# Advanced-Vision-and-Learning-Lab/sparse-view-3dgs-pack

Hardware: AMD Instinct MI355X
Metric: train-step views/s (fwd+bwd) @1M Gaussians 1080p (higher is better)
Workload: dtype f32

## Files before the change

profiles/summarize.py:

```python
#!/usr/bin/env python3
import collections
import csv
import glob
import json
import os
import sys

src, tag = sys.argv[1], sys.argv[2]
script_dir = os.path.dirname(os.path.abspath(__file__))
here = sys.argv[3] if len(sys.argv) > 3 else script_dir
sys.path.insert(0, script_dir)
from source_id import source_id


def run_identity():
    ident = {"tag": tag, "source_id": source_id(os.path.dirname(script_dir))}
    try:
        line = [x for x in open(os.path.join(src, "bench_trace.json")).read().splitlines() if x.startswith("{")][-1]
        j = json.loads(line)
        ident["P"] = j["config"]["gaussians"]
        ident["R"] = j["config"]["num_rendered_last_view"]
        ident["workload"] = j["config"]["workload"]
    except Exception as e:
        ident["identity_error"] = repr(e)
    return ident
OURS = ("preprocess_fwd_kernel", "scan_block_sums_kernel", "rs_hist_kernel", "rs_scatter_kernel", "scan_reduce_kernel",
        "scan_sums_kernel", "scan_down_kernel", "rs_rowscan_kernel", "sorted_block_sums_kernel", "duplicate_kernel", "tile_ranges_kernel",
        "bin_prepare_kernel", "render_fwd_wave_kernel", "render_bwd_wave_kernel", "render_fwd_kernel", "render_bwd_kernel", "adam_kernel", "scan_small_kernel", "preprocess_bwd_kernel", "l1_fwd_kernel",
        "l1_bwd_kernel", "dwt2_l1_fwd_kernel", "dwt2_l1_bwd_kernel", "ssim_fwd_kernel", "ssim_bwd_kernel",
        "patch_dwt_kernel", "lgdwt_combine_kernel", "act_fwd_kernel", "act_bwd_kernel", "densify_stats_kernel", "patch_means_kernel", "elf_low_kernel", "bilinear_up_kernel", "knn_search_kernel", "preprocess_bwd_step_kernel",
        "tile_order_kernel", "zero_rows_kernel", "stop_depth_bounds_kernel", "region_bin_kernel", "region_prepare_kernel",
        "status_tag_kernel", "rs_small_sort_kernel", "step_uninstanced_kernel", "chain_kernel",
        "tb_entries_kernel", "tb_emit_kernel", "tb_regions_from_counts_kernel", "tb_regions_kernel", "tb_tile_count_kernel",
        "tb_region_scan_kernel", "tb_tile_scan_kernel", "tb_write_kernel", "depth_l1_kernel", "rows_pack_kernel", "row_mask_kernel",
        "ssim_fwd_clamp_kernel", "lgdwt_bwd_kernel")


def short(name):
    for o in sorted(OURS, key=len, reverse=True):
        if o in name:
            return o
    return name.split("(")[0][-60:]


stats = glob.glob(os.path.join(src, "trace", "*", "*_kernel_stats.csv"))[0]
rows = list(csv.DictReader(open(stats)))
import shutil
shutil.copyfile(stats, os.path.join(here, "%s_rocprofv3_kernel_stats_full.csv" % tag))
with open(os.path.join(here, "%s_kernel_stats.csv" % tag), "w") as f:
    w = csv.writer(f)
    w.writerow(["Name", "Calls", "TotalDurationNs", "AverageNs", "Percentage", "MinNs", "MaxNs"])
    for r in rows[:40]:
        w.writerow([short(r["Name"]), r["Calls"], r["TotalDurationNs"], r["AverageNs"], r["Percentage"], r["MinNs"], r["MaxNs"]])

trace = glob.glob(os.path.join(src, "trace", "*", "*_kernel_trace.csv"))[0]
tr = sorted(csv.DictReader(open(trace)), key=lambda r: int(r["Start_Timestamp"]))
idx = [i for i, r in enumerate(tr) if "render_bwd_wave_kernel" in r["Kernel_Name"] or "render_bwd_kernel" in r["Kernel_Name"]]
a, b = idx[-3], idx[-2]
for j in range(len(idx) - 2, 0, -1):
    if any("step_uninstanced_kernel" in r["Kernel_Name"] for r in tr[idx[j - 1]:idx[j]]):
        a, b = idx[j - 1], idx[j]
        break
seg = tr[a:b]
wall = (int(tr[b]["Start_Timestamp"]) - int(seg[0]["Start_Timestamp"])) / 1e6
t_end = int(tr[b]["Start_Timestamp"])
iv = sorted((int(r["Start_Timestamp"]), min(int(r["End_Timestamp"]), t_end)) for r in seg)
busy, cur_s, cur_e = 0.0, None, None
for s0, e0 in iv:
    if cur_e is None or s0 > cur_e:
        if cur_e is not None:
            busy += cur_e - cur_s
        cur_s, cur_e = s0, e0
    else:
        cur_e = max(cur_e, e0)
busy = (busy + (cur_e - cur_s if cur_e is not None else 0)) / 1e6
agg = collections.OrderedDict()
for r in seg:
    n = short(r["Kernel_Name"])
    agg.setdefault(n, [0.0, 0])
    agg[n][0] += (int(r["End_Timestamp"]) - int(r["Start_Timestamp"])) / 1e3
    agg[n][1] += 1
with open(os.path.join(here, "%s_step_timeline.txt" % tag), "w") as f:
    f.write("one steady-state train step (render_bwd to render_bwd), rocprofv3 --kernel-trace\n")
    f.write("wall %.3f ms, GPU busy %.3f ms, %d kernel launches\n" % (wall, busy, len(seg)))
    for n, (d, c) in sorted(agg.items(), key=lambda x: -x[1][0]):
        f.write("%10.1f us %4d  %s\n" % (d, c, n))

traffic = {}
table = collections.defaultdict(lambda: {"FETCH_SIZE": [], "WRITE_SIZE": []})
for kind in ("fetch", "write"):
    files = glob.glob(os.path.join(src, kind, "*", "*_counter_collection.csv"))
    if not files:
        continue
    for r in csv.DictReader(open(files[0])):
        table[short(r["Kernel_Name"])][r["Counter_Name"]].append(float(r["Counter_Value"]))
with open(os.path.join(here, "%s_pmc_traffic.csv" % tag), "w") as f:
    w = csv.writer(f)
    w.writerow(["kernel", "launches", "FETCH_SIZE_KiB_mean", "WRITE_SIZE_KiB_mean", "hbm_read_bytes_corrected(x2)",
                "hbm_write_bytes", "hbm_total_bytes_per_launch"])
    for k, v in sorted(table.items()):
        if k not in OURS or not v["FETCH_SIZE"]:
            continue
        fs = v["FETCH_SIZE"][-max(1, len(v["FETCH_SIZE"]) // 3):]
        ws = v["WRITE_SIZE"][-max(1, len(v["WRITE_SIZE"]) // 3):] if v["WRITE_SIZE"] else [0.0]
        fm, wm = sum(fs) / len(fs), sum(ws) / len(ws)
        rd, wr = 2.0 * fm * 1024.0, wm * 1024.0
        w.writerow([k, len(v["FETCH_SIZE"]), "%.1f" % fm, "%.1f" % wm, "%.0f" % rd, "%.0f" % wr, "%.0f" % (rd + wr)])
        traffic[k] = rd + wr
stage_of = {"render_bwd": "render_bwd_wave_kernel", "render_fwd": "render_fwd_wave_kernel", "preprocess_fwd": "preprocess_fwd_kernel",
            "preprocess_bwd": "preprocess_bwd_kernel", "preprocess_bwd_step": "preprocess_bwd_step_kernel",
            "duplicate": "duplicate_kernel", "tile_ranges": "tile_ranges_kernel", "region_bin": "region_bin_kernel",
            "ssim_fwd": "ssim_fwd_kernel", "ssim_bwd": "ssim_bwd_kernel",
            "step_uninstanced": "step_uninstanced_kernel", "chain": "chain_kernel"}
for st, kn in (("ssim_fwd", "ssim_fwd_clamp_kernel"), ("ssim_bwd", "lgdwt_bwd_kernel")):
    if kn in traffic:
        stage_of[st] = kn
out = {st: traffic[k] for st, k in stage_of.items() if k in traffic}
out.update(run_identity())
out["launches_counted"] = {st: len(table[k]["FETCH_SIZE"]) for st, k in stage_of.items() if k in traffic}
if "region_bin_kernel" in traffic:
    out["sort"] = traffic["region_bin_kernel"]
elif "rs_scatter_kernel" in traffic:
    out["sort"] = 6 * (traffic.get("rs_scatter_kernel", 0) + traffic.get("rs_hist_kernel", 0))
json.dump(out, open(os.path.join(here, "pmc_traffic.json"), "w"), indent=1)
print(open(os.path.join(here, "%s_step_timeline.txt" % tag)).read())
print(open(os.path.join(here, "%s_pmc_traffic.csv" % tag)).read())

sq = collections.defaultdict(lambda: collections.defaultdict(list))
for f in glob.glob(os.path.join(src, "sq[0-9]*", "*", "*_counter_collection.csv")):
    for r in csv.DictReader(open(f)):
        sq[short(r["Kernel_Name"])][r["Counter_Name"]].append(float(r["Counter_Value"]))
if sq:
    with open(os.path.join(here, "%s_sq_counters.csv" % tag), "w") as f:
        w = csv.writer(f)
        w.writerow(["kernel", "waves", "VALU_insts_per_wave", "LDS_insts_per_wave", "SALU_insts_per_wave", "VMEM_rd_per_wave",
                    "VMEM_wr_per_wave", "VALU_issue_pct_of_peak", "VALU_active_x4_pct_of_SIMD_cycles", "wait_any_pct_of_wave_cycles",
                    "wait_inst_pct_of_wave_cycles", "waves_per_SIMD", "LDS_bank_conflict_pct_of_LDS_cycles"])
        sq_insts = run_identity()
        sq_insts["launches_counted"] = {}
        for k, v in sorted(sq.items()):
            m = {c: sum(x) / len(x) for c, x in v.items()}
            if k not in OURS or "GRBM_GUI_ACTIVE" not in m or m.get("SQ_WAVES", 0) == 0:
                continue
            simd_cycles = m["GRBM_GUI_ACTIVE"] / 8 * 1024
            wc = max(1.0, m.get("SQ_WAVE_CYCLES", 0))
            w.writerow([k, int(m["SQ_WAVES"]), round(m.get("SQ_INSTS_VALU", 0) / m["SQ_WAVES"], 1),
                        round(m.get("SQ_INSTS_LDS", 0) / m["SQ_WAVES"], 1), round(m.get("SQ_INSTS_SALU", 0) / m["SQ_WAVES"], 1),
                        round(m.get("SQ_INSTS_VMEM_RD", 0) / m["SQ_WAVES"], 1), round(m.get("SQ_INSTS_VMEM_WR", 0) / m["SQ_WAVES"], 1),
                        round(100 * m.get("SQ_INSTS_VALU", 0) * 2 / simd_cycles, 1),
                        round(100 * m.get("SQ_ACTIVE_INST_VALU", 0) * 4 / simd_cycles, 1),
                        round(100 * m.get("SQ_WAIT_ANY", 0) / wc, 1), round(100 * m.get("SQ_WAIT_INST_ANY", 0) / wc, 1),
                        round(wc * 4 / simd_cycles, 2),
                        round(100 * m.get("SQ_LDS_BANK_CONFLICT", 0) / max(1.0, m.get("SQ_LDS_IDX_ACTIVE", 0)), 1)])
            for st, kn in (("render_bwd", "render_bwd_wave_kernel"), ("render_fwd", "render_fwd_wave_kernel")):
                if k == kn:
                    sq_insts[st] = m.get("SQ_INSTS_VALU", 0)
                    sq_insts["launches_counted"][st] = len(v.get("SQ_INSTS_VALU", []))
                    sq_insts[st + "_valu_active_cycles_per_simd"] = m.get("SQ_ACTIVE_INST_VALU", 0) * 4 / 1024
                    sq_insts[st + "_valu_active_share_under_profiler"] = m.get("SQ_ACTIVE_INST_VALU", 0) * 4 / simd_cycles
    json.dump(sq_insts, open(os.path.join(here, "sq_insts.json"), "w"), indent=1)
    print(open(os.path.join(here, "%s_sq_counters.csv" % tag)).read())


for kind in ("init_like",):
    st_files = glob.glob(os.path.join(src, "trace_" + kind, "*", "*_kernel_stats.csv"))
    if not st_files:
        continue
# ... 66 lines not shown
```

sparse-view-3dgs-pack_amd/csrc/gs_loss.hip:

```cpp
#include "gs_common.h"
#include "gs_prof.h"

#define HC 0.7071067811865476f

struct Bands {
  float ll, lh, hl, hh;
};
__device__ __forceinline__ Bands haar_block(float a, float b, float c, float d) {
  const float lo_t = HC * a + HC * b, hi_t = HC * a - HC * b;
  const float lo_b = HC * c + HC * d, hi_b = HC * c - HC * d;
  Bands r;
  r.ll = HC * lo_t + HC * lo_b;
  r.lh = HC * lo_t - HC * lo_b;
  r.hl = HC * hi_t + HC * hi_b;
  r.hh = HC * hi_t - HC * hi_b;
  return r;
}
__device__ __forceinline__ void haar_block_adj(float gll, float glh, float ghl, float ghh, float& da, float& db,
                                               float& dc, float& dd) {
  const float dlo_t = HC * gll + HC * glh, dlo_b = HC * gll - HC * glh;
  const float dhi_t = HC * ghl + HC * ghh, dhi_b = HC * ghl - HC * ghh;
  da = HC * dlo_t + HC * dhi_t;
  db = HC * dlo_t - HC * dhi_t;
  dc = HC * dlo_b + HC * dhi_b;
  dd = HC * dlo_b - HC * dhi_b;
}
__device__ __forceinline__ float sgnf(float x) { return (float)((x > 0.f) - (x < 0.f)); }
__device__ __forceinline__ int cdiv2(int n) { return (n + 1) >> 1; }

template <int N>
__device__ __forceinline__ void block_sum_atomic(float (&v)[N], float* out) {
  __shared__ float red[GS_BLOCK / 64][N];
#pragma unroll
  for (int k = 0; k < N; k++) {
    float x = v[k];
#pragma unroll
    for (int off = 32; off >= 1; off >>= 1) x += __shfl_down(x, off, 64);
    if ((threadIdx.x & 63) == 0) red[threadIdx.x >> 6][k] = x;
  }
  __syncthreads();
  if (threadIdx.x < N) {
    float s = 0.f;
    for (int w = 0; w < GS_BLOCK / 64; w++) s += red[w][threadIdx.x];
    if (s != 0.f) atomicAdd(&out[threadIdx.x], s);
  }
}

__global__ void __launch_bounds__(GS_BLOCK) l1_fwd_kernel(const float* __restrict__ a, const float* __restrict__ b,
                                                          int64_t n, float* sum, float* __restrict__ partials) {
  float acc[1] = {0.f};
  const int64_t n4 = n >> 2;
  const float4* a4 = reinterpret_cast<const float4*>(a);
// ... 92 lines not shown
    } else if (!py && pxp) {
      p[(size_t)y0 * W + x0] = da + db;
      p[(size_t)(y0 + 1) * W + x0] = dc + dd;
    } else {
      p[(size_t)y0 * W + x0] = ((da + db) + dc) + dd;
    }
  }
}

struct Px44 {
  float v[4][4];
};
struct Blk44 {
  float l1[2][2][4];
  float l2[4];
};
template <bool FAST>
__device__ __forceinline__ void load_px44(const float* __restrict__ p, int H, int W, int i2, int j2, int h1, int w1,
                                          Px44& o) {
  if (FAST) {
#pragma unroll
    for (int y = 0; y < 4; y++) {
      const float4 q = reinterpret_cast<const float4*>(p + (size_t)(4 * i2 + y) * W)[j2];
      o.v[y][0] = q.x; o.v[y][1] = q.y; o.v[y][2] = q.z; o.v[y][3] = q.w;
    }
  } else {
#pragma unroll
    for (int r = 0; r < 2; r++)
#pragma unroll
      for (int c = 0; c < 2; c++) {
        const int r1 = min(2 * i2 + r, h1 - 1), c1 = min(2 * j2 + c, w1 - 1);
        const int y0 = 2 * r1, y1 = min(2 * r1 + 1, H - 1), x0 = 2 * c1, x1 = min(2 * c1 + 1, W - 1);
        o.v[2 * r][2 * c] = p[(size_t)y0 * W + x0];
        o.v[2 * r][2 * c + 1] = p[(size_t)y0 * W + x1];
        o.v[2 * r + 1][2 * c] = p[(size_t)y1 * W + x0];
        o.v[2 * r + 1][2 * c + 1] = p[(size_t)y1 * W + x1];
      }
  }
}
__device__ __forceinline__ void bands_of(const Px44& x, Blk44& o) {
  float ll[2][2];
#pragma unroll
  for (int r = 0; r < 2; r++)
#pragma unroll
    for (int c = 0; c < 2; c++) {
      const Bands b = haar_block(x.v[2 * r][2 * c], x.v[2 * r][2 * c + 1], x.v[2 * r + 1][2 * c], x.v[2 * r + 1][2 * c + 1]);
      o.l1[r][c][0] = b.ll; o.l1[r][c][1] = b.lh; o.l1[r][c][2] = b.hl; o.l1[r][c][3] = b.hh;
      ll[r][c] = b.ll;
    }
  const Bands b2 = haar_block(ll[0][0], ll[0][1], ll[1][0], ll[1][1]);
  o.l2[0] = b2.ll; o.l2[1] = b2.lh; o.l2[2] = b2.hl; o.l2[3] = b2.hh;
}

template <bool FAST>
__global__ void __launch_bounds__(GS_BLOCK) dwt2_l1_fwd_kernel(const float* __restrict__ pred, const float* __restrict__ gt,
                                                               int C, int H, int W, float* band_sums, float* l1_sum,
                                                               float* __restrict__ clamped_out,
                                                               const uint8_t* __restrict__ patch_mask, int ps,
                                                               float* patch_sums, float* __restrict__ partials, int clamp) {
  const int h1 = cdiv2(H), w1 = cdiv2(W), h2 = cdiv2(h1), w2 = cdiv2(w1);
  const int64_t total = (int64_t)C * h2 * w2;
  const int pnx = patch_mask ? W / ps : 0, pny = patch_mask ? H / ps : 0;
  float s[12] = {0, 0, 0, 0, 0, 0, 0, 0, 0, 0, 0, 0};
  for (int64_t o = (int64_t)blockIdx.x * GS_BLOCK + threadIdx.x; o < total; o += (int64_t)gridDim.x * GS_BLOCK) {
    const int j2 = (int)(o % w2), i2 = (int)((o / w2) % h2), c = (int)(o / ((int64_t)w2 * h2));
    Px44 pa, pb;
    load_px44<FAST>(pred + (size_t)c * H * W, H, W, i2, j2, h1, w1, pa);
    load_px44<FAST>(gt + (size_t)c * H * W, H, W, i2, j2, h1, w1, pb);
    if (FAST && (clamped_out || clamp)) {
#pragma unroll
      for (int y = 0; y < 4; y++) {
#pragma unroll
        for (int x = 0; x < 4; x++) pa.v[y][x] = fminf(fmaxf(pa.v[y][x], 0.f), 1.f);
        if (clamped_out)
          reinterpret_cast<float4*>(clamped_out + (size_t)c * H * W + (size_t)(4 * i2 + y) * W)[j2] =
              make_float4(pa.v[y][0], pa.v[y][1], pa.v[y][2], pa.v[y][3]);
      }
    }
    Blk44 a, b;
    bands_of(pa, a);
    bands_of(pb, b);
    bool in_patch = false;
    if (FAST && patch_mask) {
      const int py = (4 * i2) / ps, px = (4 * j2) / ps;
      in_patch = py < pny && px < pnx && patch_mask[py * pnx + px] != 0;
    }
#pragma unroll
    for (int r = 0; r < 2; r++)
#pragma unroll
      for (int cc = 0; cc < 2; cc++)
        if (FAST || (2 * i2 + r < h1 && 2 * j2 + cc < w1)) {
#pragma unroll
          for (int k = 0; k < 4; k++) {
            const float d = fabsf(a.l1[r][cc][k] - b.l1[r][cc][k]);
            s[k] += d;
            if (FAST && k > 0 && in_patch) s[8 + k] += d;
          }
        }
#pragma unroll
    for (int k = 0; k < 4; k++) s[4 + k] += fabsf(a.l2[k] - b.l2[k]);
    if (l1_sum) {
#pragma unroll
      for (int y = 0; y < 4; y++)
#pragma unroll
        for (int x = 0; x < 4; x++)
          if (FAST || (4 * i2 + y < H && 4 * j2 + x < W)) s[8] += fabsf(pa.v[y][x] - pb.v[y][x]);
    }
  }
  if (l1_sum) {
    __shared__ float red12[GS_BLOCK / 64][12];
#pragma unroll
    for (int k = 0; k < 12; k++) {
      float x = s[k];
#pragma unroll
      for (int off = 32; off >= 1; off >>= 1) x += __shfl_down(x, off, 64);
      if ((threadIdx.x & 63) == 0) red12[threadIdx.x >> 6][k] = x;
    }
    __syncthreads();
    if (threadIdx.x < 12) {
      float t = 0.f;
      for (int w = 0; w < GS_BLOCK / 64; w++) t += red12[w][threadIdx.x];
      if (partials)
        partials[(size_t)blockIdx.x * 12 + threadIdx.x] = t;
      else if (t != 0.f)
        atomicAdd(threadIdx.x < 8 ? &band_sums[threadIdx.x] : (threadIdx.x == 8 ? l1_sum : &patch_sums[threadIdx.x - 9]), t);
    }
  } else {
    float s8[8];
#pragma unroll
    for (int k = 0; k < 8; k++) s8[k] = s[k];
    block_sum_atomic<8>(s8, band_sums);
  }
}

template <bool FAST>
__global__ void __launch_bounds__(GS_BLOCK) dwt2_l1_bwd_kernel(const float* __restrict__ pred, const float* __restrict__ gt,
                                                               int C, int H, int W, const float* __restrict__ coef,
                                                               const float* __restrict__ l1_coef, float* __restrict__ grad,
                                                               int accumulate, const uint8_t* __restrict__ patch_mask, int ps,
                                                               const float* __restrict__ patch_coef) {
  const int h1 = cdiv2(H), w1 = cdiv2(W), h2 = cdiv2(h1), w2 = cdiv2(w1);
  const int64_t total = (int64_t)C * h2 * w2;
  const int pnx = patch_mask ? W / ps : 0, pny = patch_mask ? H / ps : 0;
  float cfg[8];
#pragma unroll
  for (int k = 0; k < 8; k++) cfg[k] = coef[k];
  float cp[3] = {0.f, 0.f, 0.f};
  if (patch_mask) { cp[0] = patch_coef[0]; cp[1] = patch_coef[1]; cp[2] = patch_coef[2]; }
  const float c1l = l1_coef ? l1_coef[0] : 0.f;
  for (int64_t o = (int64_t)blockIdx.x * GS_BLOCK + threadIdx.x; o < total; o += (int64_t)gridDim.x * GS_BLOCK) {
    const int j2 = (int)(o % w2), i2 = (int)((o / w2) % h2), c = (int)(o / ((int64_t)w2 * h2));
    Px44 pa, pb;
    load_px44<FAST>(pred + (size_t)c * H * W, H, W, i2, j2, h1, w1, pa);
    load_px44<FAST>(gt + (size_t)c * H * W, H, W, i2, j2, h1, w1, pb);
    Blk44 a, b;
    bands_of(pa, a);
    bands_of(pb, b);
    float cf[8];
#pragma unroll
    for (int k = 0; k < 8; k++) cf[k] = cfg[k];
    if (FAST && patch_mask) {
      const int py = (4 * i2) / ps, px = (4 * j2) / ps;
      if (py < pny && px < pnx && patch_mask[py * pnx + px] != 0) {
        cf[1] += cp[0];
        cf[2] += cp[1];
        cf[3] += cp[2];
      }
    }
    float dl[2][2];
    {
      float da, db, dc, dd;
      haar_block_adj(cf[4] * sgnf(a.l2[0] - b.l2[0]), cf[5] * sgnf(a.l2[1] - b.l2[1]), cf[6] * sgnf(a.l2[2] - b.l2[2]),
                     cf[7] * sgnf(a.l2[3] - b.l2[3]), da, db, dc, dd);
      const bool pr = !FAST && 2 * i2 + 1 >= h1, pc = !FAST && 2 * j2 + 1 >= w1;
      dl[0][0] = da; dl[0][1] = db; dl[1][0] = dc; dl[1][1] = dd;
      if (pr && pc) { dl[0][0] = ((da + db) + dc) + dd; }
      else if (pr) { dl[0][0] = da + dc; dl[0][1] = db + dd; }
      else if (pc) { dl[0][0] = da + db; dl[1][0] = dc + dd; }
    }
    float* gp = grad + (size_t)c * H * W;
    float out[4][4];
#pragma unroll
    for (int r = 0; r < 2; r++)
#pragma unroll
      for (int cc = 0; cc < 2; cc++) {
// ... 93 lines not shown

template <bool BWD>
__global__ void __launch_bounds__(GS_BLOCK) patch_dwt_kernel(const float* __restrict__ pred, const float* __restrict__ gt,
                                                             int C, int H, int W, int ps, const uint8_t* __restrict__ mask,
                                                             float* sums, const float* __restrict__ coef,
                                                             float* __restrict__ grad) {
  const int patch = blockIdx.x;
  if (!mask[patch]) return;
  const int nx = W / ps, hp = cdiv2(ps);
  const int px = patch % nx, py = patch / nx;
  const int total = C * hp * hp;
  float s[3] = {0.f, 0.f, 0.f};
  float cf0 = 0.f, cf1 = 0.f, cf2 = 0.f;
  if (BWD) { cf0 = coef[0]; cf1 = coef[1]; cf2 = coef[2]; }
  for (int o = blockIdx.y * GS_BLOCK + threadIdx.x; o < total; o += gridDim.y * GS_BLOCK) {
    const int j = o % hp, i = (o / hp) % hp, c = o / (hp * hp);
    const int y0 = py * ps + 2 * i, x0 = px * ps + 2 * j;
    const bool pyb = 2 * i + 1 >= ps, pxb = 2 * j + 1 >= ps;
    const int y1 = pyb ? y0 : y0 + 1, x1 = pxb ? x0 : x0 + 1;
    const float* p = pred + (size_t)c * H * W;
    const float* q = gt + (size_t)c * H * W;
    const Bands a = haar_block(p[(size_t)y0 * W + x0], p[(size_t)y0 * W + x1], p[(size_t)y1 * W + x0], p[(size_t)y1 * W + x1]);
    const Bands b = haar_block(q[(size_t)y0 * W + x0], q[(size_t)y0 * W + x1], q[(size_t)y1 * W + x0], q[(size_t)y1 * W + x1]);
    if (!BWD) {
      s[0] += fabsf(a.lh - b.lh);
      s[1] += fabsf(a.hl - b.hl);
      s[2] += fabsf(a.hh - b.hh);
    } else {
      float da, db, dc, dd;
      haar_block_adj(0.f, cf0 * sgnf(a.lh - b.lh), cf1 * sgnf(a.hl - b.hl), cf2 * sgnf(a.hh - b.hh), da, db, dc, dd);
      float* g = grad + (size_t)c * H * W;
      float v00 = da, v01 = db, v10 = dc, v11 = dd;
      if (pyb && pxb) v00 = ((da + db) + dc) + dd;
      else if (pyb) { v00 = da + dc; v01 = db + dd; }
      else if (pxb) { v00 = da + db; v10 = dc + dd; }
      g[(size_t)y0 * W + x0] += v00;
      if (!pxb) g[(size_t)y0 * W + x1] += v01;
      if (!pyb) { g[(size_t)y1 * W + x0] += v10; if (!pxb) g[(size_t)y1 * W + x1] += v11; }
    }
  }
  if (!BWD) block_sum_atomic<3>(s, sums);
}

__constant__ float GW[11] = {0.001028380123898387f, 0.0075987582094967365f, 0.036000773310661316f,
                             0.10936068743467331f,  0.21300552785396576f,  0.26601171493530273f,
                             0.21300552785396576f,  0.10936068743467331f,  0.036000773310661316f,
                             0.0075987582094967365f, 0.001028380123898387f};
#define ST 32
#define SH (ST + 10)

#define HS 33

struct SsimTile { int bx, by, z, linear; bool live; };
__device__ __forceinline__ SsimTile ssim_tile_of_block(int gx, int gy, int gz) {
  const int n = gx * gy * gz, per = (n + 7) / 8;
  const int t = (int)(blockIdx.x & 7) * per + (int)(blockIdx.x >> 3);
  SsimTile r;
  r.live = (int)(blockIdx.x >> 3) < per && t < n;
  r.linear = t;
  r.z = t / (gx * gy);
  const int rem = t - r.z * gx * gy;
  r.by = (rem / gx) * ST;
  r.bx = (rem % gx) * ST;
  return r;
}
static inline unsigned ssim_launch_blocks(int W, int H, int planes) {
  const int n = ((W + ST - 1) / ST) * ((H + ST - 1) / ST) * planes;
  return (unsigned)(((n + 7) / 8) * 8);
}

template <int NQ, bool FWD>
__device__ __forceinline__ void ssim_conv_tile(const float (*tile)[SH][SH + 1], float (*hor)[SH][HS], float (&out)[4][NQ]) {
#pragma clang fp contract(fast)
  constexpr int NITEM = SH * (ST / 4);
  constexpr int NR = (NITEM + GS_BLOCK - 1) / GS_BLOCK;
  float acc[NR][4][NQ];
#pragma unroll
  for (int rd = 0; rd < NR; rd++) {
    const int item = threadIdx.x + rd * GS_BLOCK;
#pragma unroll
    for (int j = 0; j < 4; j++)
#pragma unroll
      for (int q = 0; q < NQ; q++) acc[rd][j][q] = 0.f;
    if (item < NITEM) {
      const int r = item / (ST / 4), c0 = (item % (ST / 4)) * 4;
#pragma unroll
      for (int e = 0; e < 14; e++) {
        float val[NQ];
        if (FWD) {
          const float a = tile[0][r][c0 + e], b = tile[1][r][c0 + e];
          val[0] = a; val[1] = a * a; val[2] = b; val[3 % NQ] = b * b; val[4 % NQ] = a * b;
        } else {
#pragma unroll
          for (int q = 0; q < NQ; q++) val[q] = tile[q][r][c0 + e];
        }
#pragma unroll
        for (int j = 0; j < 4; j++) {
          const int t = e - j;
          if (t >= 0 && t < 11) {
#pragma unroll
            for (int q = 0; q < NQ; q++) acc[rd][j][q] += GW[t] * val[q];
          }
        }
      }
    }
  }
  __syncthreads();
#pragma unroll
  for (int rd = 0; rd < NR; rd++) {
    const int item = threadIdx.x + rd * GS_BLOCK;
    if (item < NITEM) {
      const int r = item / (ST / 4), c0 = (item % (ST / 4)) * 4;
#pragma unroll
      for (int j = 0; j < 4; j++)
#pragma unroll
        for (int q = 0; q < NQ; q++) hor[q][r][c0 + j] = acc[rd][j][q];
    }
  }
// ... 209 lines not shown
#pragma unroll
    for (int it = 0; it < NIT; it++) {
      const int k = threadIdx.x + it * GS_BLOCK;
      if (k < SH * SH) {
        tile[0][k / SH][k % SH] = a[it] * g[it];
        tile[1][k / SH][k % SH] = b[it] * g[it];
        tile[2][k / SH][k % SH] = d[it] * g[it];
      }
    }
  }
}

__global__ void __launch_bounds__(GS_BLOCK) ssim_bwd_kernel(const float* __restrict__ img1, const float* __restrict__ img2,
                                                            int H, int W, const float* __restrict__ dL_dmap,
                                                            const float* __restrict__ dm_dmu1,
                                                            const float* __restrict__ dm_dsigma1_sq,
                                                            const float* __restrict__ dm_dsigma12,
                                                            float* __restrict__ dL_dimg1, const float* __restrict__ coef_dev,
                                                            int accumulate, const float* __restrict__ clamp_src, int planes) {
  constexpr int LDS_WORDS = (3 * SH * (SH + 1) > 3 * SH * HS) ? 3 * SH * (SH + 1) : 3 * SH * HS;
  __shared__ float lds_buf[LDS_WORDS];
  float (*tile)[SH][SH + 1] = reinterpret_cast<float (*)[SH][SH + 1]>(lds_buf);
  float (*hor)[SH][HS] = reinterpret_cast<float (*)[SH][HS]>(lds_buf);
  const float gu = coef_dev ? coef_dev[0] : 0.f;
  const SsimTile tl = ssim_tile_of_block((W + ST - 1) / ST, (H + ST - 1) / ST, planes);
  if (!tl.live) return;
  const size_t plane = (size_t)tl.z * H * W;
  const int bx = tl.bx, by = tl.by;
  ssim_stage_bwd(dL_dmap, gu, dm_dmu1, dm_dsigma1_sq, dm_dsigma12, plane, H, W, bx, by, tile);
  __syncthreads();
  float out[4][3];
  ssim_conv_tile<3, false>(tile, hor, out);
  const int lx = threadIdx.x & 31, ly0 = threadIdx.x >> 5;
#pragma unroll
  for (int m = 0; m < 4; m++) {
    const int x = bx + lx, y = by + 4 * ly0 + m;
    if (x >= W || y >= H) continue;
    const size_t o = plane + (size_t)y * W + x;
    const float r = clamp_src ? clamp_src[o] : 0.f;
    const float a1 = clamp_src ? (r < 0.f ? 0.f : (r > 1.f ? 1.f : r)) : img1[o];
    float dL = 0.0f;
    dL += out[m][0];
    dL += a1 * 2.0f * out[m][1];
    dL += img2[o] * out[m][2];
    if (accumulate) dL += dL_dimg1[o];
    if (clamp_src && (r < 0.f || r > 1.f)) dL = 0.f;
    dL_dimg1[o] = dL;
  }
}

#define LGDWT_CLAMP 1
#define LGDWT_DWT 2
#define LGDWT_CLAMP_MASK 4
__global__ void __launch_bounds__(GS_BLOCK) ssim_fwd_clamp_kernel(const float* __restrict__ raw, const float* __restrict__ gt,
                                                                  int H, int W, int planes, float C1, float C2,
                                                                  float* __restrict__ dm_dmu1, float* __restrict__ dm_dsigma1_sq,
                                                                  float* __restrict__ dm_dsigma12, float* __restrict__ partials) {
  constexpr int LDS_WORDS = (2 * SH * (SH + 1) > 5 * SH * HS) ? 2 * SH * (SH + 1) : 5 * SH * HS;
  __shared__ float lds_buf[LDS_WORDS];
  float (*tile)[SH][SH + 1] = reinterpret_cast<float (*)[SH][SH + 1]>(lds_buf);
  float (*hor)[SH][HS] = reinterpret_cast<float (*)[SH][HS]>(lds_buf);
  const SsimTile tl = ssim_tile_of_block((W + ST - 1) / ST, (H + ST - 1) / ST, planes);
  if (!tl.live) return;
  const size_t plane = (size_t)tl.z * H * W;
  const int bx = tl.bx, by = tl.by;
  ssim_stage_fwd(raw, gt, plane, H, W, bx, by, true, tile);
  __syncthreads();
  float out[4][5];
  ssim_conv_tile<5, true>(tile, hor, out);
  const float msum = ssim_fwd_pixels(out, plane, H, W, bx, by, C1, C2, nullptr, dm_dmu1, dm_dsigma1_sq, dm_dsigma12);
  ssim_store_partial(msum, partials, tl.linear);
}

__device__ __forceinline__ void dwt2_l1_adjoint_col(const float (&a)[4], const float (&b)[4], int c4, const float (&cf)[8],
                                                    float c1l, float (&g)[4]) {
  float pa[4], pb[4];
#pragma unroll
  for (int m = 0; m < 4; m++) {
    pa[m] = __shfl_xor(a[m], 1, 64);
    pb[m] = __shfl_xor(b[m], 1, 64);
  }
  const bool right = (c4 & 1) != 0, cc = (c4 & 2) != 0;
  Bands A[2], B[2];
#pragma unroll
  for (int r = 0; r < 2; r++) {
    A[r] = haar_block(right ? pa[2 * r] : a[2 * r], right ? a[2 * r] : pa[2 * r], right ? pa[2 * r + 1] : a[2 * r + 1],
                      right ? a[2 * r + 1] : pa[2 * r + 1]);
    B[r] = haar_block(right ? pb[2 * r] : b[2 * r], right ? b[2 * r] : pb[2 * r], right ? pb[2 * r + 1] : b[2 * r + 1],
                      right ? b[2 * r + 1] : pb[2 * r + 1]);
  }
  float la[2][2], lb[2][2];
#pragma unroll
  for (int r = 0; r < 2; r++) {
    const float oa = __shfl_xor(A[r].ll, 2, 64), ob = __shfl_xor(B[r].ll, 2, 64);
    la[r][0] = cc ? oa : A[r].ll;
    la[r][1] = cc ? A[r].ll : oa;
    lb[r][0] = cc ? ob : B[r].ll;
    lb[r][1] = cc ? B[r].ll : ob;
  }
  const Bands a2 = haar_block(la[0][0], la[0][1], la[1][0], la[1][1]);
  const Bands b2 = haar_block(lb[0][0], lb[0][1], lb[1][0], lb[1][1]);
  float da, db, dc, dd;
  haar_block_adj(cf[4] * sgnf(a2.ll - b2.ll), cf[5] * sgnf(a2.lh - b2.lh), cf[6] * sgnf(a2.hl - b2.hl),
                 cf[7] * sgnf(a2.hh - b2.hh), da, db, dc, dd);
#pragma unroll
  for (int r = 0; r < 2; r++) {
    const float dl = r == 0 ? (cc ? db : da) : (cc ? dd : dc);
    float ea, eb, ec, ed;
    haar_block_adj(cf[0] * sgnf(A[r].ll - B[r].ll) + dl, cf[1] * sgnf(A[r].lh - B[r].lh), cf[2] * sgnf(A[r].hl - B[r].hl),
                   cf[3] * sgnf(A[r].hh - B[r].hh), ea, eb, ec, ed);
    g[2 * r] = right ? eb : ea;
    g[2 * r + 1] = right ? ed : ec;
  }
#pragma unroll
  for (int m = 0; m < 4; m++) g[m] += c1l * sgnf(a[m] - b[m]);
}

__global__ void __launch_bounds__(GS_BLOCK) __attribute__((amdgpu_waves_per_eu(7))) lgdwt_bwd_kernel(const float* __restrict__ raw, const float* __restrict__ gt, int H,
                                                             int W, int planes, int flags, const uint8_t* __restrict__ patch_mask,
                                                             int ps, const float* __restrict__ coef,
                                                             const float* __restrict__ dm_dmu1,
                                                             const float* __restrict__ dm_dsigma1_sq,
                                                             const float* __restrict__ dm_dsigma12, float* __restrict__ grad) {
  constexpr int LDS_WORDS = (3 * SH * (SH + 1) > 3 * SH * HS) ? 3 * SH * (SH + 1) : 3 * SH * HS;
// ... 441 lines not shown
    loss = loss + p.patch_weight * patch;
  }
  out[0] = loss; out[1] = base; out[2] = dwt; out[3] = patch; out[4] = scale; out[5] = l1; out[6] = ssim;
  out[8] = w_l1 / p.n_pix;
  out[9] = -w_ssim / p.n_pix;
  if (p.reset_sums) {
    float* z = const_cast<float*>(sums_in);
    for (int k = 0; k < 13; k++) z[k] = 0.f;
  }
}

int gs_lgdwt_combine_pp(const float* sums, const float* ssim_partials, int64_t n_partials, const float* dwt_partials,
                        int64_t n_dwt, const float* l1_partials, int64_t n_l1, float* running_mean, const GsLgdwtParams* p,
                        float* out, void* stream) {
  if (!sums || !running_mean || !p || !out) return GS_E_NULL;
  if (n_partials < 0 || n_partials > 0x7FFFFFFF || (n_partials > 0 && !ssim_partials)) return GS_E_SHAPE;
  if (n_dwt < 0 || n_dwt > 65536 || (n_dwt > 0 && !dwt_partials) || n_l1 < 0 || n_l1 > 65536 || (n_l1 > 0 && !l1_partials))
    return GS_E_SHAPE;
  hipStream_t s = (hipStream_t)stream;
  (void)hipGetLastError();
  hipLaunchKernelGGL(lgdwt_combine_kernel, dim3(1), dim3(1024), 0, s, sums, running_mean, *p, out, ssim_partials,
                     (int)n_partials, dwt_partials, (int)n_dwt, l1_partials, (int)n_l1);
  GS_LAUNCH_CHECK(s, 0);
  return GS_OK;
}
int gs_lgdwt_combine_p(const float* sums, const float* ssim_partials, int64_t n_partials, float* running_mean,
                       const GsLgdwtParams* p, float* out, void* stream) {
  return gs_lgdwt_combine_pp(sums, ssim_partials, n_partials, nullptr, 0, nullptr, 0, running_mean, p, out, stream);
}
int gs_lgdwt_combine(const float* sums, float* running_mean, const GsLgdwtParams* p, float* out, void* stream) {
  return gs_lgdwt_combine_p(sums, nullptr, 0, running_mean, p, out, stream);
}

static inline bool lgdwt_fused_ok(const void* a, const void* b, const void* c, const void* d, const void* e, int32_t C, int32_t H,
                                  int32_t W) {
  return (H % 4) == 0 && (W % 4) == 0 && C <= 65535 &&
         ((((uintptr_t)a | (uintptr_t)b | (uintptr_t)c | (uintptr_t)d | (uintptr_t)e) & 15) == 0);
}
static inline int lgdwt_fused_args(int32_t C, int32_t H, int32_t W, int32_t ps, const uint8_t* mask) {
  if (C <= 0 || H <= 0 || W <= 0 || ps < 0) return GS_E_SHAPE;
  if ((ps > 0) != (mask != nullptr)) return GS_E_NULL;
  if (ps > 0 && (H < ps || W < ps)) return GS_E_SHAPE;
  if (ps % 4 != 0) return GS_E_UNSUPPORTED;
  return GS_OK;
}
int gs_lgdwt_fused_fwd(const float* raw, const float* gt, int32_t C, int32_t H, int32_t W, float C1, float C2, int32_t ps,
                       const uint8_t* mask, float* dwt_partials, float* ssim_partials, float* dm_dmu1, float* dm_dsigma1_sq,
                       float* dm_dsigma12, void* stream) {
  if (!raw || !gt || !dwt_partials || !ssim_partials || !dm_dmu1 || !dm_dsigma1_sq || !dm_dsigma12) return GS_E_NULL;
  const int rc = lgdwt_fused_args(C, H, W, ps, mask);
  if (rc != GS_OK) return rc;
  if (!lgdwt_fused_ok(raw, gt, dm_dmu1, dm_dsigma1_sq, dm_dsigma12, C, H, W)) return GS_E_UNSUPPORTED;
  hipStream_t s = (hipStream_t)stream;
  {
    GS_PROF(ST_DWT2_FWD, s);
    float dummy_target = 0.f;
    const int r = dwt2_l1_fwd_launch(raw, gt, C, H, W, &dummy_target, &dummy_target, s, nullptr, mask, ps, &dummy_target,
                                     dwt_partials, true);
    if (r != GS_OK) return r;
  }
  GS_PROF(ST_SSIM_FWD, s);
  hipLaunchKernelGGL(ssim_fwd_clamp_kernel, dim3(ssim_launch_blocks(W, H, C)), dim3(GS_BLOCK), 0, s, raw, gt, H, W, C, C1, C2,
                     dm_dmu1, dm_dsigma1_sq, dm_dsigma12, ssim_partials);
  GS_LAUNCH_CHECK(s, 0);
  return GS_OK;
}
int gs_lgdwt_fused_bwd(const float* raw, const float* gt, int32_t C, int32_t H, int32_t W, int32_t flags, int32_t ps,
                       const uint8_t* mask, const float* coef_dev, const float* dm_dmu1, const float* dm_dsigma1_sq,
                       const float* dm_dsigma12, float* grad, void* stream) {
  if (!raw || !gt || !coef_dev || !dm_dmu1 || !dm_dsigma1_sq || !dm_dsigma12 || !grad) return GS_E_NULL;
  const int rc = lgdwt_fused_args(C, H, W, ps, mask);
  if (rc != GS_OK) return rc;
  if (!lgdwt_fused_ok(raw, gt, dm_dmu1, dm_dsigma1_sq, dm_dsigma12, C, H, W) || ((uintptr_t)grad & 15) != 0)
    return GS_E_UNSUPPORTED;
  hipStream_t s = (hipStream_t)stream;
  GS_PROF(ST_SSIM_BWD, s);
  hipLaunchKernelGGL(lgdwt_bwd_kernel, dim3(ssim_launch_blocks(W, H, C)), dim3(GS_BLOCK), 0, s, raw, gt, H, W, C, flags, mask, ps,
                     coef_dev, dm_dmu1, dm_dsigma1_sq, dm_dsigma12, grad);
  GS_LAUNCH_CHECK(s, 0);
  return GS_OK;
}
}
```

Before: 1173.

## Fuse DWT L1 forward and SSIM forward into one interleaved launch

```diff
diff --git a/profiles/summarize.py b/profiles/summarize.py
--- a/profiles/summarize.py
+++ b/profiles/summarize.py
@@ -33,7 +33,7 @@
         "status_tag_kernel", "rs_small_sort_kernel", "step_uninstanced_kernel", "chain_kernel",
         "tb_entries_kernel", "tb_emit_kernel", "tb_regions_from_counts_kernel", "tb_regions_kernel", "tb_tile_count_kernel",
         "tb_region_scan_kernel", "tb_tile_scan_kernel", "tb_write_kernel", "depth_l1_kernel", "rows_pack_kernel", "row_mask_kernel",
-        "ssim_fwd_clamp_kernel", "lgdwt_bwd_kernel")
+        "ssim_fwd_clamp_kernel", "lgdwt_bwd_kernel", "lgdwt_fwd_kernel")
 
 
 def short(name):
@@ -112,7 +112,7 @@
             "duplicate": "duplicate_kernel", "tile_ranges": "tile_ranges_kernel", "region_bin": "region_bin_kernel",
             "ssim_fwd": "ssim_fwd_kernel", "ssim_bwd": "ssim_bwd_kernel",
             "step_uninstanced": "step_uninstanced_kernel", "chain": "chain_kernel"}
-for st, kn in (("ssim_fwd", "ssim_fwd_clamp_kernel"), ("ssim_bwd", "lgdwt_bwd_kernel")):
+for st, kn in (("ssim_fwd", "ssim_fwd_clamp_kernel"), ("ssim_fwd", "lgdwt_fwd_kernel"), ("ssim_bwd", "lgdwt_bwd_kernel")):
     if kn in traffic:
         stage_of[st] = kn
 out = {st: traffic[k] for st, k in stage_of.items() if k in traffic}
diff --git a/sparse-view-3dgs-pack_amd/csrc/gs_loss.hip b/sparse-view-3dgs-pack_amd/csrc/gs_loss.hip
--- a/sparse-view-3dgs-pack_amd/csrc/gs_loss.hip
+++ b/sparse-view-3dgs-pack_amd/csrc/gs_loss.hip
@@ -1,3 +1,5 @@
+#include <cstdlib>
+
 #include "gs_common.h"
 #include "gs_prof.h"
 
@@ -196,17 +198,17 @@
   o.l2[0] = b2.ll; o.l2[1] = b2.lh; o.l2[2] = b2.hl; o.l2[3] = b2.hh;
 }
 
-template <bool FAST>
-__global__ void __launch_bounds__(GS_BLOCK) dwt2_l1_fwd_kernel(const float* __restrict__ pred, const float* __restrict__ gt,
-                                                               int C, int H, int W, float* band_sums, float* l1_sum,
-                                                               float* __restrict__ clamped_out,
-                                                               const uint8_t* __restrict__ patch_mask, int ps,
-                                                               float* patch_sums, float* __restrict__ partials, int clamp) {
+template <bool FAST, bool ROWS>
+__device__ __forceinline__ void dwt2_l1_fwd_body(const float* __restrict__ pred, const float* __restrict__ gt, int C, int H,
+                                                 int W, float* band_sums, float* l1_sum, float* __restrict__ clamped_out,
+                                                 const uint8_t* __restrict__ patch_mask, int ps, float* patch_sums,
+                                                 float* __restrict__ partials, int clamp, unsigned wg, unsigned nwg,
+                                                 float (*red12)[12]) {
   const int h1 = cdiv2(H), w1 = cdiv2(W), h2 = cdiv2(h1), w2 = cdiv2(w1);
   const int64_t total = (int64_t)C * h2 * w2;
   const int pnx = patch_mask ? W / ps : 0, pny = patch_mask ? H / ps : 0;
   float s[12] = {0, 0, 0, 0, 0, 0, 0, 0, 0, 0, 0, 0};
-  for (int64_t o = (int64_t)blockIdx.x * GS_BLOCK + threadIdx.x; o < total; o += (int64_t)gridDim.x * GS_BLOCK) {
+  for (int64_t o = (int64_t)wg * GS_BLOCK + threadIdx.x; o < total; o += (int64_t)nwg * GS_BLOCK) {
     const int j2 = (int)(o % w2), i2 = (int)((o / w2) % h2), c = (int)(o / ((int64_t)w2 * h2));
     Px44 pa, pb;
     load_px44<FAST>(pred + (size_t)c * H * W, H, W, i2, j2, h1, w1, pa);
@@ -243,7 +245,7 @@
         }
 #pragma unroll
     for (int k = 0; k < 4; k++) s[4 + k] += fabsf(a.l2[k] - b.l2[k]);
-    if (l1_sum) {
+    if (ROWS || l1_sum) {
 #pragma unroll
       for (int y = 0; y < 4; y++)
 #pragma unroll
@@ -251,8 +253,7 @@
           if (FAST || (4 * i2 + y < H && 4 * j2 + x < W)) s[8] += fabsf(pa.v[y][x] - pb.v[y][x]);
     }
   }
-  if (l1_sum) {
-    __shared__ float red12[GS_BLOCK / 64][12];
+  if (ROWS || l1_sum) {
 #pragma unroll
     for (int k = 0; k < 12; k++) {
       float x = s[k];
@@ -264,8 +265,8 @@
     if (threadIdx.x < 12) {
       float t = 0.f;
       for (int w = 0; w < GS_BLOCK / 64; w++) t += red12[w][threadIdx.x];
-      if (partials)
-        partials[(size_t)blockIdx.x * 12 + threadIdx.x] = t;
+      if (ROWS || partials)
+        partials[(size_t)wg * 12 + threadIdx.x] = t;
       else if (t != 0.f)
         atomicAdd(threadIdx.x < 8 ? &band_sums[threadIdx.x] : (threadIdx.x == 8 ? l1_sum : &patch_sums[threadIdx.x - 9]), t);
     }
@@ -275,6 +276,16 @@
     for (int k = 0; k < 8; k++) s8[k] = s[k];
     block_sum_atomic<8>(s8, band_sums);
   }
+}
+template <bool FAST>
+__global__ void __launch_bounds__(GS_BLOCK) dwt2_l1_fwd_kernel(const float* __restrict__ pred, const float* __restrict__ gt,
+                                                               int C, int H, int W, float* band_sums, float* l1_sum,
+                                                               float* __restrict__ clamped_out,
+                                                               const uint8_t* __restrict__ patch_mask, int ps,
+                                                               float* patch_sums, float* __restrict__ partials, int clamp) {
+  __shared__ float red12[GS_BLOCK / 64][12];
+  dwt2_l1_fwd_body<FAST, false>(pred, gt, C, H, W, band_sums, l1_sum, clamped_out, patch_mask, ps, patch_sums, partials, clamp,
+                         blockIdx.x, gridDim.x, red12);
 }
 
 template <bool FAST>
@@ -474,11 +485,11 @@
 #define HS 33
 
 struct SsimTile { int bx, by, z, linear; bool live; };
-__device__ __forceinline__ SsimTile ssim_tile_of_block(int gx, int gy, int gz) {
+__device__ __forceinline__ SsimTile ssim_tile_of_block(int gx, int gy, int gz, unsigned b) {
   const int n = gx * gy * gz, per = (n + 7) / 8;
-  const int t = (int)(blockIdx.x & 7) * per + (int)(blockIdx.x >> 3);
+  const int t = (int)(b & 7) * per + (int)(b >> 3);
   SsimTile r;
-  r.live = (int)(blockIdx.x >> 3) < per && t < n;
+  r.live = (int)(b >> 3) < per && t < n;
   r.linear = t;
   r.z = t / (gx * gy);
   const int rem = t - r.z * gx * gy;
@@ -486,6 +497,7 @@
   r.bx = (rem % gx) * ST;
   return r;
 }
+__device__ __forceinline__ SsimTile ssim_tile_of_block(int gx, int gy, int gz) { return ssim_tile_of_block(gx, gy, gz, blockIdx.x); }
 static inline unsigned ssim_launch_blocks(int W, int H, int planes) {
   const int n = ((W + ST - 1) / ST) * ((H + ST - 1) / ST) * planes;
   return (unsigned)(((n + 7) / 8) * 8);
@@ -801,15 +813,14 @@
 #define LGDWT_CLAMP 1
 #define LGDWT_DWT 2
 #define LGDWT_CLAMP_MASK 4
-__global__ void __launch_bounds__(GS_BLOCK) ssim_fwd_clamp_kernel(const float* __restrict__ raw, const float* __restrict__ gt,
-                                                                  int H, int W, int planes, float C1, float C2,
-                                                                  float* __restrict__ dm_dmu1, float* __restrict__ dm_dsigma1_sq,
-                                                                  float* __restrict__ dm_dsigma12, float* __restrict__ partials) {
-  constexpr int LDS_WORDS = (2 * SH * (SH + 1) > 5 * SH * HS) ? 2 * SH * (SH + 1) : 5 * SH * HS;
-  __shared__ float lds_buf[LDS_WORDS];
+constexpr int SSIM_FWD_LDS_WORDS = (2 * SH * (SH + 1) > 5 * SH * HS) ? 2 * SH * (SH + 1) : 5 * SH * HS;
+__device__ __forceinline__ void ssim_fwd_clamp_body(const float* __restrict__ raw, const float* __restrict__ gt, int H, int W,
+                                                    int planes, float C1, float C2, float* __restrict__ dm_dmu1,
+                                                    float* __restrict__ dm_dsigma1_sq, float* __restrict__ dm_dsigma12,
+                                                    float* __restrict__ partials, unsigned b, float* lds_buf) {
   float (*tile)[SH][SH + 1] = reinterpret_cast<float (*)[SH][SH + 1]>(lds_buf);
   float (*hor)[SH][HS] = reinterpret_cast<float (*)[SH][HS]>(lds_buf);
-  const SsimTile tl = ssim_tile_of_block((W + ST - 1) / ST, (H + ST - 1) / ST, planes);
+  const SsimTile tl = ssim_tile_of_block((W + ST - 1) / ST, (H + ST - 1) / ST, planes, b);
   if (!tl.live) return;
   const size_t plane = (size_t)tl.z * H * W;
   const int bx = tl.bx, by = tl.by;
@@ -819,6 +830,47 @@
   ssim_conv_tile<5, true>(tile, hor, out);
   const float msum = ssim_fwd_pixels(out, plane, H, W, bx, by, C1, C2, nullptr, dm_dmu1, dm_dsigma1_sq, dm_dsigma12);
   ssim_store_partial(msum, partials, tl.linear);
+}
+__global__ void __launch_bounds__(GS_BLOCK) ssim_fwd_clamp_kernel(const float* __restrict__ raw, const float* __restrict__ gt,
+                                                                  int H, int W, int planes, float C1, float C2,
+                                                                  float* __restrict__ dm_dmu1, float* __restrict__ dm_dsigma1_sq,
+                                                                  float* __restrict__ dm_dsigma12, float* __restrict__ partials) {
+  __shared__ float lds_buf[SSIM_FWD_LDS_WORDS];
+  ssim_fwd_clamp_body(raw, gt, H, W, planes, C1, C2, dm_dmu1, dm_dsigma1_sq, dm_dsigma12, partials, blockIdx.x, lds_buf);
+}
+
+__global__ void __launch_bounds__(GS_BLOCK) lgdwt_fwd_kernel(const float* __restrict__ raw, const float* __restrict__ gt, int C,
+                                                             int H, int W, float C1, float C2,
+                                                             const uint8_t* __restrict__ patch_mask, int ps,
+                                                             float* __restrict__ dwt_partials, unsigned n_dwt, unsigned dwt_every,
+                                                             float* __restrict__ dm_dmu1, float* __restrict__ dm_dsigma1_sq,
+                                                             float* __restrict__ dm_dsigma12, float* __restrict__ ssim_partials) {
+  static_assert(SSIM_FWD_LDS_WORDS >= (GS_BLOCK / 64) * 12, "red12 lives in the SSIM tile buffer");
+  __shared__ float lds_buf[SSIM_FWD_LDS_WORDS];
+  const unsigned row = blockIdx.x >> 3, lane8 = blockIdx.x & 7, dwt_rows = (n_dwt + 7) >> 3;
+  bool is_dwt;
+  unsigned sub_row;
+  if (dwt_every == 0) {
+    is_dwt = row < dwt_rows;
+    sub_row = is_dwt ? row : row - dwt_rows;
+  } else {
+    const unsigned period = row / (dwt_every + 1), q = row % (dwt_every + 1);
+    if (period < dwt_rows) {
+      is_dwt = q == 0;
+      sub_row = is_dwt ? period : period * dwt_every + (q - 1);
+    } else {
+      is_dwt = false;
+      sub_row = row - dwt_rows;
+    }
+  }
+  const unsigned b = sub_row * 8 + lane8;
+  if (is_dwt) {
+    if (b >= n_dwt) return;
+    dwt2_l1_fwd_body<true, true>(raw, gt, C, H, W, dwt_partials, dwt_partials, nullptr, patch_mask, ps, dwt_partials,
+                                 dwt_partials, 1, b, n_dwt, reinterpret_cast<float (*)[12]>(lds_buf));
+  } else {
+    ssim_fwd_clamp_body(raw, gt, H, W, C, C1, C2, dm_dmu1, dm_dsigma1_sq, dm_dsigma12, ssim_partials, b, lds_buf);
+  }
 }
 
 __device__ __forceinline__ void dwt2_l1_adjoint_col(const float (&a)[4], const float (&b)[4], int c4, const float (&cf)[8],
@@ -1366,16 +1418,27 @@
   if (rc != GS_OK) return rc;
   if (!lgdwt_fused_ok(raw, gt, dm_dmu1, dm_dsigma1_sq, dm_dsigma12, C, H, W)) return GS_E_UNSUPPORTED;
   hipStream_t s = (hipStream_t)stream;
-  {
-    GS_PROF(ST_DWT2_FWD, s);
-    float dummy_target = 0.f;
-    const int r = dwt2_l1_fwd_launch(raw, gt, C, H, W, &dummy_target, &dummy_target, s, nullptr, mask, ps, &dummy_target,
-                                     dwt_partials, true);
-    if (r != GS_OK) return r;
-  }
+  static const bool split = [] { const char* e = getenv("GS_LGDWT_FWD_SPLIT"); return e && atoi(e) != 0; }();
+  if (split) {
+    {
+      GS_PROF(ST_DWT2_FWD, s);
+      float dummy_target = 0.f;
+      const int r = dwt2_l1_fwd_launch(raw, gt, C, H, W, &dummy_target, &dummy_target, s, nullptr, mask, ps, &dummy_target,
+                                       dwt_partials, true);
+      if (r != GS_OK) return r;
+    }
+    GS_PROF(ST_SSIM_FWD, s);
+    hipLaunchKernelGGL(ssim_fwd_clamp_kernel, dim3(ssim_launch_blocks(W, H, C)), dim3(GS_BLOCK), 0, s, raw, gt, H, W, C, C1, C2,
+                       dm_dmu1, dm_dsigma1_sq, dm_dsigma12, ssim_partials);
+    GS_LAUNCH_CHECK(s, 0);
+    return GS_OK;
+  }
+  const unsigned n_ssim = ssim_launch_blocks(W, H, C), n_dwt = dwt2_fwd_workgroups(C, H, W);
+  const unsigned ssim_rows = n_ssim / 8, dwt_rows = (n_dwt + 7) / 8;
+  const unsigned every = ssim_rows / dwt_rows < 4 ? ssim_rows / dwt_rows : 4;
   GS_PROF(ST_SSIM_FWD, s);
-  hipLaunchKernelGGL(ssim_fwd_clamp_kernel, dim3(ssim_launch_blocks(W, H, C)), dim3(GS_BLOCK), 0, s, raw, gt, H, W, C, C1, C2,
-                     dm_dmu1, dm_dsigma1_sq, dm_dsigma12, ssim_partials);
+  hipLaunchKernelGGL(lgdwt_fwd_kernel, dim3((ssim_rows + dwt_rows) * 8), dim3(GS_BLOCK), 0, s, raw, gt, C, H, W, C1, C2, mask, ps,
+                     dwt_partials, n_dwt, every, dm_dmu1, dm_dsigma1_sq, dm_dsigma12, ssim_partials);
   GS_LAUNCH_CHECK(s, 0);
   return GS_OK;
 }
```

Result: faster. 1186 (median of 6 runs) (+1.1%).
